# danilobellini/audiolazy

Hardware: NVIDIA H100
Metric: samples/sec through 64-ch gammatone bank (higher is better)
Workload: dtype f64

## Files before the change

### audiolazy_b200/csrc/alz_capi.cu

```cuda
#pragma GCC visibility push(default)
#include "../../include/alz_b200.h"
#pragma GCC visibility pop
#include "alz_biquad.cuh"
#include "alz_generic.cuh"
#include "alz_lane_tma.cuh"
#include "alz_plan.h"

#include <algorithm>
#include <cctype>
#include <cmath>
#include <cstring>
#include <map>
#include <thread>

#include <sys/mman.h>
#include <sys/syscall.h>
#include <unistd.h>

static std::mutex g_host_mu;
static std::map<void*, size_t> g_host_allocs;

static_assert(ALZI_OK == ALZ_OK && ALZI_ERR_CUDA == ALZ_ERR_CUDA && ALZI_ERR_UNSUPPORTED == ALZ_ERR_UNSUPPORTED, "status codes");

static thread_local std::string g_err;
std::atomic<long long> alzi_launches{0};
#define g_launches alzi_launches

int alzi_fail(int code, const char* fmt, ...) {
  char buf[512];
  va_list ap;
  va_start(ap, fmt);
  vsnprintf(buf, sizeof buf, fmt, ap);
  va_end(ap);
  g_err = buf;
  return code;
}
#define fail alzi_fail

int alzi_env_int(const char* name, int dflt) {
  const char* v = getenv(name);
  return (v && *v) ? atoi(v) : dflt;
}
#define env_int alzi_env_int

static double env_double(const char* name, double dflt) {
  const char* v = getenv(name);
  return (v && *v) ? atof(v) : dflt;
}

void alzi_keep_async_pool() {
  static std::once_flag once[64];
  int dev = 0;
  cudaGetDevice(&dev);
  std::call_once(once[dev & 63], [dev] {
    cudaMemPool_t pool;
    if (cudaDeviceGetDefaultMemPool(&pool, dev) == cudaSuccess) {
      unsigned long long keep = ~0ull;
      cudaMemPoolSetAttribute(pool, cudaMemPoolAttrReleaseThreshold, &keep);
    }
    cudaGetLastError();
  });
}
#define keep_async_pool alzi_keep_async_pool

static const int kCoefSmall = 512, kCoefLarge = 3584;

__global__ void __launch_bounds__(32)
alz_generic_kernel(const __grid_constant__ AlzTileArgs a, const __grid_constant__ AlzGenericArgs ca) {
  extern __shared__ __align__(16) float alz_smem[];
  alz_run_warp<AlzGenericCore>(a, ca, alz_smem);
}

__global__ void __launch_bounds__(32)
alz_generic_tma_kernel(const __grid_constant__ AlzTileArgs a, const __grid_constant__ AlzGenericArgs ca,
                       const __grid_constant__ CUtensorMap tmx, const __grid_constant__ CUtensorMap tmy) {
  extern __shared__ __align__(1024) unsigned char alz_smem_tma[];
  alz_run_warp_tma<AlzGenericCore>(a, ca, &tmx, &tmy, alz_smem_tma);
}

typedef CUresult (*alz_encode_tiled_fn)(CUtensorMap*, CUtensorMapDataType, cuuint32_t, void*, const cuuint64_t*,
                                        const cuuint64_t*, const cuuint32_t*, const cuuint32_t*, CUtensorMapInterleave,
                                        CUtensorMapSwizzle, CUtensorMapL2promotion, CUtensorMapFloatOOBfill);
static alz_encode_tiled_fn get_encode_tiled() {
  static alz_encode_tiled_fn fn = nullptr;
  static std::once_flag once;
  std::call_once(once, [] {
    void* p = nullptr;
    cudaDriverEntryPointQueryResult q;
    if (cudaGetDriverEntryPoint("cuTensorMapEncodeTiled", &p, cudaEnableDefault, &q) == cudaSuccess &&
        q == cudaDriverEntryPointSuccess)
      fn = (alz_encode_tiled_fn)p;
    cudaGetLastError();
  });
  return fn;
}

template <class F>
static bool driver_fn(const char* name, F* out) {
  void* p = nullptr;
  cudaDriverEntryPointQueryResult q;
  if (cudaGetDriverEntryPoint(name, &p, cudaEnableDefault, &q) != cudaSuccess || q != cudaDriverEntryPointSuccess || !p) {
    cudaGetLastError();
    return false;
  }
  *out = (F)p;
  return true;
}
static std::map<void*, CUgreenCtx> g_partitions;

bool alzi_make_tensor_maps(const AlzTileArgs& ta, CUtensorMap* tmx, CUtensorMap* tmy) {
  alz_encode_tiled_fn enc = get_encode_tiled();
  if (!enc || !ta.vec_in || !ta.vec_out || env_int("ALZ_NO_TMA", 0)) return false;
  if (ta.T >= (1ll << 31) || ta.S >= (1ll << 31)) return false;
  if ((unsigned long long)ta.xs * 4 >= (1ull << 40) || (unsigned long long)ta.ysS * 4 >= (1ull << 40)) return false;
  if (ta.ysS & 3) return false;
  const cuuint32_t estr[4] = {1, 1, 1, 1};
  if (ta.vP > 0) {
    const cuuint64_t P = (cuuint64_t)ta.vP, Sreal = (cuuint64_t)(ta.S / ta.vP);
    const cuuint64_t xdims[3] = {(cuuint64_t)ta.T, P, Sreal};
    const cuuint64_t xstr[2] = {(cuuint64_t)ta.T * 4, (cuuint64_t)ta.xs * 4};
    const cuuint32_t xbox[3] = {32, 32, 1};
    if (enc(tmx, CU_TENSOR_MAP_DATA_TYPE_FLOAT32, 3, (void*)ta.x, xdims, xstr, xbox, estr, CU_TENSOR_MAP_INTERLEAVE_NONE,
            CU_TENSOR_MAP_SWIZZLE_128B, CU_TENSOR_MAP_L2_PROMOTION_L2_128B, CU_TENSOR_MAP_FLOAT_OOB_FILL_NONE) != CUDA_SUCCESS)
      return false;
    const cuuint64_t ydims[4] = {(cuuint64_t)ta.T, P, (cuuint64_t)ta.C, Sreal};
    const cuuint64_t ystr[3] = {(cuuint64_t)ta.T * 4, (cuuint64_t)ta.ys * 4, (cuuint64_t)ta.ysS * 4};
    const cuuint32_t ybox[4] = {32, 32, 1, 1};
    return enc(tmy, CU_TENSOR_MAP_DATA_TYPE_FLOAT32, 4, (void*)ta.y, ydims, ystr, ybox, estr, CU_TENSOR_MAP_INTERLEAVE_NONE,
               CU_TENSOR_MAP_SWIZZLE_128B, CU_TENSOR_MAP_L2_PROMOTION_NONE, CU_TENSOR_MAP_FLOAT_OOB_FILL_NONE) == CUDA_SUCCESS;
  }
  {
    const cuuint64_t dims[3] = {(cuuint64_t)ta.T, (cuuint64_t)ta.S, 1};
    const cuuint64_t strides[2] = {(cuuint64_t)ta.xs * 4, (cuuint64_t)ta.xs * 4};
    const cuuint32_t box[3] = {32, 32, 1};
    if (enc(tmx, CU_TENSOR_MAP_DATA_TYPE_FLOAT32, 3, (void*)ta.x, dims, strides, box, estr, CU_TENSOR_MAP_INTERLEAVE_NONE,
            CU_TENSOR_MAP_SWIZZLE_128B, CU_TENSOR_MAP_L2_PROMOTION_L2_128B, CU_TENSOR_MAP_FLOAT_OOB_FILL_NONE) != CUDA_SUCCESS)
      return false;
  }
  {
    const cuuint64_t dims[4] = {(cuuint64_t)ta.T, (cuuint64_t)ta.C, (cuuint64_t)ta.S, 1};
    const cuuint64_t strides[3] = {(cuuint64_t)ta.ys * 4, (cuuint64_t)ta.ysS * 4, (cuuint64_t)ta.ysS * 4};
    const cuuint32_t box[4] = {32, 1, 32, 1};
    if (enc(tmy, CU_TENSOR_MAP_DATA_TYPE_FLOAT32, 4, (void*)ta.y, dims, strides, box, estr, CU_TENSOR_MAP_INTERLEAVE_NONE,
            CU_TENSOR_MAP_SWIZZLE_128B, CU_TENSOR_MAP_L2_PROMOTION_NONE, CU_TENSOR_MAP_FLOAT_OOB_FILL_NONE) != CUDA_SUCCESS)
      return false;
  }
  return true;
}

static bool make_map_2d(const float* ptr, long long T, long long n_rows, long long stride, CUtensorMap* tm) {
  alz_encode_tiled_fn enc = get_encode_tiled();
  if (!enc || ((uintptr_t)ptr & 15) || (stride & 3) || T >= (1ll << 31) || n_rows >= (1ll << 31)) return false;
  const cuuint32_t estr[2] = {1, 1};
  const cuuint64_t dims[2] = {(cuuint64_t)T, (cuuint64_t)n_rows};
  const cuuint64_t strides[1] = {(cuuint64_t)stride * 4};
  const cuuint32_t box[2] = {32, 32};
  return enc(tm, CU_TENSOR_MAP_DATA_TYPE_FLOAT32, 2, (void*)ptr, dims, strides, box, estr, CU_TENSOR_MAP_INTERLEAVE_NONE,
             CU_TENSOR_MAP_SWIZZLE_128B, CU_TENSOR_MAP_L2_PROMOTION_L2_128B, CU_TENSOR_MAP_FLOAT_OOB_FILL_NONE) == CUDA_SUCCESS;
}

static int launch_biquad(const alz_plan* p, const AlzTileArgs& ta, cudaStream_t st) {
  if (p->NB0 == 8) {
    if (p->K == 1) return alzi_launch_headfir_k1(p, ta, st);
    if (p->K == 4) return alzi_launch_headfir_k4(p, ta, st);
    return fail(ALZ_ERR_UNSUPPORTED, "no head-FIR kernel for K=%d", p->K);
  }
  switch (p->K) {
    case 1: return alzi_launch_biquad_k1(p, ta, st);
    case 2: return alzi_launch_biquad_k2(p, ta, st);
    case 3: return alzi_launch_biquad_k3(p, ta, st);
    case 4: return alzi_launch_biquad_k4(p, ta, st);
    case 6: return alzi_launch_biquad_k6(p, ta, st);
    case 8: return alzi_launch_biquad_k8(p, ta, st);
  }
  return fail(ALZ_ERR_UNSUPPORTED, "no biquad kernel for K=%d", p->K);
}

static double probe_biquad(const alz_plan* p, const double* r64, const double* r32) {
  if (p->NB0 == 8) return p->K == 1 ? alzi_probe_headfir_k1(p, r64, r32) : alzi_probe_headfir_k4(p, r64, r32);
  switch (p->K) {
    case 1: return alzi_probe_biquad_k1(p, r64, r32);
    case 2: return alzi_probe_biquad_k2(p, r64, r32);
    case 3: return alzi_probe_biquad_k3(p, r64, r32);
    case 4: return alzi_probe_biquad_k4(p, r64, r32);
    case 6: return alzi_probe_biquad_k6(p, r64, r32);
    default: return alzi_probe_biquad_k8(p, r64, r32);
  }
}

static int launch_generic(const alz_plan* p, AlzTileArgs ta, cudaStream_t st, const double* tv = nullptr,
                          long long tv_stride = 0) {
  AlzGenericArgs ga{p->d_sec, p->d_tap_delay, p->d_coef, p->K, p->C, 0, tv, tv_stride};
  const long long groups = (ta.S + 31) / 32;
  CUtensorMap tmx, tmy;
  if (alzi_make_tensor_maps(ta, &tmx, &tmy))
    alz_generic_tma_kernel<<<dim3((unsigned)p->C, (unsigned)groups), 32, ALZ_TMA_SMEM, st>>>(ta, ga, tmx, tmy);
  else
    alz_generic_kernel<<<dim3((unsigned)p->C, (unsigned)groups), 32, ALZ_WARP_SMEM, st>>>(ta, ga);
  ALZ_CUDA(cudaGetLastError());
  g_launches.fetch_add(1, std::memory_order_relaxed);
  return ALZ_OK;
}

static const int kBiquadKs[] = {1, 2, 3, 4, 6, 8};
static const double kTierMaxRadius = 0.99;
static const double kChunkMaxErr = 2.5e-8;
static const long long kChunkProbeLen = 1024;

template <class Sec>
static double chunk_error(const std::vector<Sec>& secs, long long L) {
  const size_t K = secs.size();
  struct Hist { std::vector<std::vector<double>> x, y; };
  auto zero = [&]() {
    Hist h;
    for (const Sec& s : secs) { h.x.emplace_back(s.b.size() - 1, 0.0); h.y.emplace_back(s.a.size() - 1, 0.0); }
    return h;
  };
  auto step = [&](Hist& h, double v) {
    for (size_t k = 0; k < K; ++k) {
      const Sec& s = secs[k];
      std::vector<double>& xh = h.x[k];
      std::vector<double>& yh = h.y[k];
      double acc = s.b[0] * v;
      for (size_t j = 1; j < s.b.size(); ++j) acc += s.b[j] * xh[j - 1];
      for (size_t j = 1; j < s.a.size(); ++j) acc -= s.a[j] * yh[j - 1];
      if (!xh.empty()) { std::copy_backward(xh.begin(), xh.end() - 1, xh.end()); xh[0] = v; }
      if (!yh.empty()) { std::copy_backward(yh.begin(), yh.end() - 1, yh.end()); yh[0] = acc; }
      v = acc;
    }
    return v;
  };
  std::vector<double> x(3 * L);
  unsigned seed = 2024u;
  for (auto& v : x) { seed = seed * 1664525u + 1013904223u; v = (double)(float)((double)(seed >> 8) * (2.0 / 16777216.0) - 1.0); }
  Hist seq = zero();
  for (long long n = 0; n < L; ++n) step(seq, x[n]);
  Hist chunk = seq;
  for (long long n = 0; n < L; ++n) step(chunk, 0.0);
  Hist f = zero();
  for (long long n = L; n < 2 * L; ++n) { step(seq, x[n]); step(f, x[n]); }
  for (size_t k = 0; k < K; ++k) {
    for (size_t j = 0; j < chunk.x[k].size(); ++j) chunk.x[k][j] += f.x[k][j];
    for (size_t j = 0; j < chunk.y[k].size(); ++j) chunk.y[k][j] += f.y[k][j];
  }
  double peak = 0.0, err = 0.0;
  for (long long n = 2 * L; n < 3 * L; ++n) {
    const double want = step(seq, x[n]), got = step(chunk, x[n]);
    peak = std::max(peak, std::fabs(want));
    const double d = std::fabs(got - want);
    err = std::max(err, d == d ? d : 1e300);
  }
  return peak > 0.0 ? err / peak : (err > 0.0 ? 1e300 : 0.0);
}

extern "C" {

const char* alz_last_error(void) { return g_err.c_str(); }
int32_t alz_abi_version(void) { return ALZ_ABI_VERSION; }
int64_t alz_launch_count(void) { return g_launches.load(); }

int32_t alz_device_count(void) {
  int n = 0;
  if (cudaGetDeviceCount(&n) != cudaSuccess) { cudaGetLastError(); return 0; }
  return n;
}

int32_t alz_set_device(int32_t device) {
  ALZ_CUDA(cudaSetDevice(device));
  return ALZ_OK;
}

int32_t alz_plan_create(const double* coef, const int32_t* desc, int32_t C, int32_t KM, alz_plan** out) {
  return alz_plan_create_ex(coef, desc, C, KM, 0, out);
}

int32_t alz_plan_create_ex(const double* coef, const int32_t* desc, int32_t C, int32_t KM, int32_t flags,
                           alz_plan** out) {
  if (!out) return fail(ALZ_ERR_INVALID, "out is null");
  *out = nullptr;
  if (!coef || !desc || C <= 0 || KM < 0) return fail(ALZ_ERR_INVALID, "bad plan arguments");
  const bool design_only = (flags & ALZ_PLAN_DESIGN_ONLY) != 0;
  int dev = -1;
  if (!design_only) ALZ_CUDA(cudaGetDevice(&dev));

  struct Sec { std::vector<double> b, a; };
  std::vector<std::vector<Sec>> secs(C);
  int Kmax = 0, nbmax = 1, namax = 1;
  for (int c = 0; c < C; ++c) {
    bool ended = false;
    for (int k = 0; k < KM; ++k) {
      const int32_t* d = desc + ((size_t)c * KM + k) * 3;
      const int nb = d[0], na = d[1];
      if (nb == 0) { ended = true; continue; }
      if (ended) return fail(ALZ_ERR_INVALID, "channel %d: section %d follows an absent section", c, k);
      if (nb < 0 || na < 1 || d[2] < 0) return fail(ALZ_ERR_INVALID, "channel %d section %d: bad descriptor", c, k);
      const double* b = coef + d[2];
      const double* a = b + nb;
      if (a[0] == 0.0) return fail(ALZ_ERR_ZERO_GAIN, "channel %d section %d: Invalid filter gain (a0 == 0)", c, k);
      Sec s;
      s.b.assign(b, b + nb);
      s.a.assign(a, a + na);
      const double a0 = a[0];
      if (a0 != 1.0) {
        for (auto& v : s.b) v /= a0;
        for (auto& v : s.a) v /= a0;
        s.a[0] = 1.0;
      }
      while (s.b.size() > 1 && s.b.back() == 0.0) s.b.pop_back();
      while (s.a.size() > 1 && s.a.back() == 0.0) s.a.pop_back();
      for (double v : s.b) if (!std::isfinite(v)) return fail(ALZ_ERR_INVALID, "non-finite coefficient");
      for (double v : s.a) if (!std::isfinite(v)) return fail(ALZ_ERR_INVALID, "non-finite coefficient");
      nbmax = std::max(nbmax, (int)s.b.size());
      namax = std::max(namax, (int)s.a.size());
      secs[c].push_back(std::move(s));
    }
    Kmax = std::max(Kmax, (int)secs[c].size());
  }
  if (Kmax == 0) Kmax = 1;

  alz_plan* p = new (std::nothrow) alz_plan();
  if (!p) return fail(ALZ_ERR_NOMEM, "out of host memory");
  p->C = C;
  p->device = dev;
  p->sequential = (flags & ALZ_PLAN_SEQUENTIAL) != 0;
  p->parallel_sum = (flags & ALZ_PLAN_PARALLEL) != 0;
  if (design_only || cudaDeviceGetAttribute(&p->sm_count, cudaDevAttrMultiProcessorCount, dev) != cudaSuccess || p->sm_count <= 0) {
    cudaGetLastError();
    p->sm_count = 132;
  }

  p->fr_desc.assign((size_t)C * Kmax * 3, 0);
  for (int c = 0; c < C; ++c)
    for (size_t k = 0; k < secs[c].size(); ++k) {
      int* d = &p->fr_desc[((size_t)c * Kmax + k) * 3];
      d[0] = (int)secs[c][k].b.size(); d[1] = (int)secs[c][k].a.size(); d[2] = (int)p->fr_coef.size();
      p->fr_coef.insert(p->fr_coef.end(), secs[c][k].b.begin(), secs[c][k].b.end());
      p->fr_coef.insert(p->fr_coef.end(), secs[c][k].a.begin(), secs[c][k].a.end());
    }
  p->fr_K = Kmax;

  int nb_first = 1, nb_rest = 1;
  for (int c = 0; c < C; ++c)
    for (size_t k = 0; k < secs[c].size(); ++k) {
      if (k == 0) nb_first = std::max(nb_first, (int)secs[c][k].b.size());
      else nb_rest = std::max(nb_rest, (int)secs[c][k].b.size());
    }
  const bool plain = nbmax <= 3 && namax <= 3 && Kmax <= 8;
  const bool headfir = !plain && namax <= 3 && nb_first <= 8 && nb_rest <= 3 && Kmax <= 4;
  const bool biquad = (plain || headfir) && !(flags & ALZ_PLAN_FORCE_GENERIC);
  if (biquad) {
    int K = 8;
    for (int kk : kBiquadKs) if (kk >= Kmax) { K = kk; break; }
    if (headfir) K = Kmax == 1 ? 1 : 4;
    p->kind = ALZ_KIND_BIQUAD;
    p->K = K;
    p->NB = headfir ? (nb_rest <= 1 ? 1 : 3) : nbmax;
    p->NB0 = headfir ? 8 : 0;
    p->xd = ALZ_H0(p->NB0); p->yd = 2;
    p->state_doubles = ALZ_STATE_SLOTS(K, p->NB0);
    bool monic = !p->parallel_sum;
    for (int c = 0; c < C && monic; ++c) {
      double g = 1.0;
      for (auto& s : secs[c]) {
        const double b0 = s.b[0];
        if (!(std::fabs(b0) > 1e-150 && std::fabs(b0) < 1e150)) { monic = false; break; }
        g *= b0;
        if (!(std::fabs(g) > 1e-250 && std::fabs(g) < 1e250)) { monic = false; break; }
      }
    }
    bool gain_in = monic && !env_int("ALZ_EXACT_GAIN", 0);
    for (int c = 0; c < C && gain_in; ++c) {
      double g = 1.0;
      for (auto& s : secs[c]) g *= s.b[0];
      if (!(std::fabs(g) > 1e-30 && std::fabs(g) < 1e30)) gain_in = false;
    }
    p->monic = monic ? (gain_in ? 2 : 1) : 0;
    p->fp64_ops = (monic ? K * (p->NB - 1 + 2) + (gain_in ? 0 : 1) : K * (p->NB + 2)) + (headfir ? 8 - p->NB : 0);
    if (!headfir && !env_int("ALZ_NO_ZMASK", 0)) {
      int zm = (1 << (2 * K)) - 1;
      for (int c = 0; c < C; ++c)
        for (size_t k = 0; k < secs[c].size(); ++k)
          for (int j = 1; j <= 2; ++j)
            if ((int)secs[c][k].b.size() > j && secs[c][k].b[j] != 0.0) zm &= ~(1 << (2 * (int)k + j - 1));
      p->zmask = zm;
      if (K == 4 && p->NB == 3 && (zm & ALZ_ZMASK_KLAPURI) == ALZ_ZMASK_KLAPURI) p->fp64_ops -= 6;
    }
    const int stride = ALZ_COEF_STRIDE(K, p->NB0), nval = ALZ_COEF_NVAL(K, p->NB0);
    std::vector<double> tab((size_t)C * stride, 0.0);
    p->sc.assign((size_t)C * (K + 1), 1.0);
    for (int c = 0; c < C; ++c) {
      double* rec = tab.data() + (size_t)c * stride;
      double g = 1.0, sc = 1.0;
      if (p->monic == 2) {
        double gg = 1.0;
        for (auto& s : secs[c]) gg *= s.b[0];
        sc = (double)(float)gg;
        p->sc[(size_t)c * (K + 1)] = sc;
      }
      for (int k = 0; k < K; ++k) {
        double b[8] = {1.0, 0, 0, 0, 0, 0, 0, 0}, a[3] = {1.0, 0.0, 0.0};
        if (k < (int)secs[c].size()) {
          const Sec& s = secs[c][k];
          b[0] = 0.0;
          for (size_t i = 0; i < s.b.size(); ++i) b[i] = s.b[i];
          for (size_t i = 0; i < s.a.size(); ++i) a[i] = s.a[i];
        }
        if (k == 0 && p->NB0 == 8)
          for (int j = 3; j < 8; ++j) rec[5 * K + 1 + (j - 3)] = monic ? b[j] / b[0] : b[j];
        if (monic) {
          rec[5 * k + 0] = 1.0;
          rec[5 * k + 1] = b[1] / b[0];
          rec[5 * k + 2] = b[2] / b[0];
          g *= b[0];
          sc /= b[0];
        } else {
          rec[5 * k + 0] = b[0];
          rec[5 * k + 1] = b[1];
          rec[5 * k + 2] = b[2];
        }
        rec[5 * k + 3] = -a[1];
        rec[5 * k + 4] = -a[2];
        p->sc[(size_t)c * (K + 1) + k + 1] = sc;
      }
      rec[5 * K] = monic ? g : 1.0;
    }
    p->tier.assign(C, 0);
    p->tier_err.assign(C, -1.0);
    p->tier_tol = env_double("ALZ_TIER_TOL", 2.5e-6);
    p->probe_len = std::max(64, env_int("ALZ_TIER_PROBE", 8192));
    const bool tiering = !(flags & ALZ_PLAN_EXACT) && !p->parallel_sum && !env_int("ALZ_NO_FP32_TIER", 0) && p->tier_tol > 0.0;
    std::vector<double> tab32((size_t)C * stride, 0.0);
    for (int c = 0; c < C; ++c) {
      const double* rec = tab.data() + (size_t)c * stride;
      float* r32 = reinterpret_cast<float*>(tab32.data() + (size_t)c * stride);
      bool representable = true;
      for (int i = 0; i < nval; ++i) {
        r32[i] = (float)rec[i];
        if (rec[i] != 0.0 && !(std::fabs(rec[i]) > 1e-30 && std::fabs(rec[i]) < 1e30)) representable = false;
      }
      double radius = 0.0;
      for (auto& s : secs[c]) {
        const double a1 = s.a.size() > 1 ? s.a[1] : 0.0, a2 = s.a.size() > 2 ? s.a[2] : 0.0, disc = a1 * a1 - 4.0 * a2;
        radius = std::max(radius, disc < 0.0 ? std::sqrt(a2) : 0.5 * (std::fabs(a1) + std::sqrt(disc)));
      }
      if (tiering && representable) {
        p->tier_err[c] = probe_biquad(p, rec, tab32.data() + (size_t)c * stride);
        if (p->tier_err[c] <= p->tier_tol && radius <= kTierMaxRadius) { p->tier[c] = 1; ++p->n_fp32; }
      }
    }
    if (!p->sequential)
      for (int c = 0; c < C; ++c) p->chunk_err = std::max(p->chunk_err, chunk_error(secs[c], kChunkProbeLen));
    {
      std::vector<int> lst[2];
      const int order = env_int("ALZ_TIER_ORDER", 1);
      for (int c = 0; c < C; ++c) lst[order == 1 ? p->tier[c] : (order == 2 ? 1 - p->tier[c] : 0)].push_back(c);
      size_t i0 = 0, i1 = 0;
      p->pos_channel.clear();
      while (i0 < lst[0].size() || i1 < lst[1].size()) {
        const bool take0 = i1 >= lst[1].size() || (i0 < lst[0].size() && i0 * lst[1].size() <= i1 * lst[0].size());
        p->pos_channel.push_back(take0 ? lst[0][i0++] : lst[1][i1++]);
      }
    }
    p->h_tab.assign((size_t)C * stride, 0.0);
    for (int pos = 0; pos < C; ++pos) {
      const int c = p->pos_channel[pos];
      const std::vector<double>& src = p->tier[c] ? tab32 : tab;
      double* rec = p->h_tab.data() + (size_t)pos * stride;
      memcpy(rec, src.data() + (size_t)c * stride, (size_t)nval * sizeof(double));
      rec[ALZ_COEF_META(K, p->NB0)] = (double)(c + 65536 * p->tier[c]);
    }
    p->fp64_ops_exact = p->fp64_ops;
    p->coef_small = C * stride <= kCoefSmall;
    const int ncoef = p->coef_small ? kCoefSmall : kCoefLarge;
    const int per_launch = ncoef / stride;
    if (per_launch < 1) { alz_plan_destroy(p); return fail(ALZ_ERR_UNSUPPORTED, "coefficient record too large"); }
    for (int p0 = 0; p0 < C; p0 += per_launch) {
      const int npos = std::min(per_launch, C - p0);
      char* blk = (char*)calloc(1, 2 * sizeof(int) + (size_t)ncoef * sizeof(double));
      if (!blk) { alz_plan_destroy(p); return fail(ALZ_ERR_NOMEM, "out of host memory"); }
      reinterpret_cast<int*>(blk)[0] = stride;
      reinterpret_cast<int*>(blk)[1] = npos;
      memcpy(blk + 2 * sizeof(int), p->h_tab.data() + (size_t)p0 * stride, (size_t)npos * stride * sizeof(double));
      p->chunks.push_back({blk, npos});
    }
    p->tile_group = env_int("ALZ_TILE_GROUP", 2);
    if (p->tile_group != 1 && p->tile_group != 2 && p->tile_group != 4) p->tile_group = 2;
  } else if (Kmax == 1 && !(flags & ALZ_PLAN_FORCE_GENERIC) && C * 32 <= kCoefLarge && !env_int("ALZ_NO_WINDOW", 0)) {
    p->kind = ALZ_KIND_GENERIC;
    p->window = true;
    p->K = 1;
    p->NB = nbmax;
    p->monic = 0;
    int near_x = 0, near_y = 0, maxd_x = 0, maxd_y = 0;
    std::vector<int> far_x, far_y;
    for (int c = 0; c < C; ++c) {
      if (secs[c].empty()) continue;
      const Sec& s = secs[c][0];
      for (size_t d = 1; d < s.b.size(); ++d)
        if (s.b[d] != 0.0) {
          maxd_x = std::max(maxd_x, (int)d);
          if (d < 16) near_x = std::max(near_x, (int)d);
          else if (std::find(far_x.begin(), far_x.end(), (int)d) == far_x.end()) far_x.push_back((int)d);
        }
      for (size_t d = 1; d < s.a.size(); ++d)
        if (s.a[d] != 0.0) {
          maxd_y = std::max(maxd_y, (int)d);
          if (d < 16) near_y = std::max(near_y, (int)d);
          else if (std::find(far_y.begin(), far_y.end(), (int)d) == far_y.end()) far_y.push_back((int)d);
        }
    }
    std::sort(far_x.begin(), far_x.end());
    std::sort(far_y.begin(), far_y.end());
    auto slots_of = [](int nearest) { return nearest == 0 ? 0 : (nearest <= 3 ? 4 : 16); };
    auto pow2 = [](int n) { int q = 1; while (q < n) q <<= 1; return q; };
    p->win_mx = slots_of(near_x);
    p->win_my = slots_of(near_y);
    p->win_nfx = (int)far_x.size();
    p->win_nfy = (int)far_y.size();
    int slot = 1;
    p->win_xwin = slot; slot += p->win_mx ? p->win_mx - 1 : 0;
    p->win_ywin = slot; slot += p->win_my ? p->win_my - 1 : 0;
    if (!far_x.empty()) { p->win_xbase = slot; p->win_xmask = pow2(far_x.back() + 16) - 1; slot += p->win_xmask + 1; }
    if (!far_y.empty()) { p->win_ybase = slot; p->win_ymask = pow2(far_y.back() + 16) - 1; slot += p->win_ymask + 1; }
    p->xd = maxd_x; p->yd = maxd_y;
    p->state_doubles = slot;
    p->fp64_ops = 1 + (p->win_mx ? p->win_mx - 1 : 0) + (p->win_my ? p->win_my - 1 : 0) + p->win_nfx + p->win_nfy;
    p->win_far_delay = far_x;
    p->win_far_delay.insert(p->win_far_delay.end(), far_y.begin(), far_y.end());
    p->h_tab.assign((size_t)C * 32, 0.0);
    std::vector<double> fcoef(std::max<size_t>(1, p->win_far_delay.size()) * C, 0.0);
    for (int c = 0; c < C; ++c) {
      double* rec = p->h_tab.data() + (size_t)c * 32;
      if (secs[c].empty()) { rec[0] = 1.0; continue; }
      const Sec& s = secs[c][0];
      for (size_t d = 0; d < s.b.size() && d < 16; ++d) rec[d] = s.b[d];
      for (size_t d = 1; d < s.a.size() && d < 16; ++d) rec[16 + d - 1] = -s.a[d];
      for (size_t f = 0; f < far_x.size(); ++f) fcoef[f * C + c] = (size_t)far_x[f] < s.b.size() ? s.b[far_x[f]] : 0.0;
      for (size_t f = 0; f < far_y.size(); ++f) fcoef[(far_x.size() + f) * C + c] = (size_t)far_y[f] < s.a.size() ? -s.a[far_y[f]] : 0.0;
    }
    p->coef_small = C * 32 <= 64;
    p->win_block = calloc(1, alzi_window_block_bytes(p->coef_small));
    if (!p->win_block) { alz_plan_destroy(p); return fail(ALZ_ERR_NOMEM, "out of host memory"); }
    if (!design_only) {
      const size_t nf = std::max<size_t>(1, p->win_far_delay.size());
      std::vector<int> fd(nf, 16);
      std::copy(p->win_far_delay.begin(), p->win_far_delay.end(), fd.begin());
      cudaError_t e = cudaMalloc(&p->d_far_delay, nf * sizeof(int));
      if (e == cudaSuccess) e = cudaMemcpy(p->d_far_delay, fd.data(), nf * sizeof(int), cudaMemcpyHostToDevice);
      if (e == cudaSuccess) e = cudaMalloc(&p->d_far_coef, fcoef.size() * sizeof(double));
      if (e == cudaSuccess) e = cudaMemcpy(p->d_far_coef, fcoef.data(), fcoef.size() * sizeof(double), cudaMemcpyHostToDevice);
      if (e != cudaSuccess) { alz_plan_destroy(p); return fail(ALZ_ERR_CUDA, "plan upload failed: %s", cudaGetErrorString(e)); }
    }
    alzi_window_block_fill(p->win_block, p->coef_small, p->win_nfx, p->win_nfy, p->win_xbase, p->win_xmask, p->win_ybase,
                           p->win_ymask, p->win_xwin, p->win_ywin, C, p->d_far_delay, p->d_far_coef, p->h_tab.data());
  } else {
    const int K = Kmax;
    p->kind = ALZ_KIND_GENERIC;
    p->K = K;
    p->NB = nbmax;
    p->monic = 0;
    std::vector<int> tap_delay;
    std::vector<std::vector<double>> tap_coef;
    p->h_sec.resize(K);
    p->h_xlen.assign(K, 0);
    p->h_ylen.assign(K, 0);
    int slot = 1;
    int ops = 0, xdmax = 0, ydmax = 0;
    for (int k = 0; k < K; ++k) {
      size_t nb = 1, na = 1;
      for (int c = 0; c < C; ++c)
        if (k < (int)secs[c].size()) { nb = std::max(nb, secs[c][k].b.size()); na = std::max(na, secs[c][k].a.size()); }
      AlzGenSection gs{};
      gs.num_begin = (int)tap_delay.size();
      for (size_t d = 0; d < nb; ++d) {
        std::vector<double> col(C, 0.0);
        bool any = false;
        for (int c = 0; c < C; ++c) {
          double v;
          if (k < (int)secs[c].size()) v = d < secs[c][k].b.size() ? secs[c][k].b[d] : 0.0;
          else v = d == 0 ? 1.0 : 0.0;
          col[c] = v;
          any = any || v != 0.0;
        }
        if (any || d == 0) { tap_delay.push_back((int)d); tap_coef.push_back(std::move(col)); p->h_tap_is_den.push_back(0); }
      }
      gs.nnum = (int)tap_delay.size() - gs.num_begin;
      gs.den_begin = (int)tap_delay.size();
      for (size_t d = 1; d < na; ++d) {
        std::vector<double> col(C, 0.0);
        bool any = false;
        for (int c = 0; c < C; ++c) {
          double v = (k < (int)secs[c].size() && d < secs[c][k].a.size()) ? -secs[c][k].a[d] : 0.0;
          col[c] = v;
          any = any || v != 0.0;
        }
        if (any) { tap_delay.push_back((int)d); tap_coef.push_back(std::move(col)); p->h_tap_is_den.push_back(1); }
      }
      gs.nden = (int)tap_delay.size() - gs.den_begin;
      const int xlen = (int)nb - 1, ylen = (int)na - 1;
      auto pow2 = [](int n) { int q = 1; while (q < n) q <<= 1; return q; };
      if (xlen > 0) { gs.xbase = slot; gs.xmask = pow2(xlen) - 1; slot += gs.xmask + 1; } else { gs.xbase = 0; gs.xmask = -1; }
      if (ylen > 0) { gs.ybase = slot; gs.ymask = pow2(ylen) - 1; slot += gs.ymask + 1; } else { gs.ybase = 0; gs.ymask = -1; }
      p->h_sec[k] = gs;
      p->h_xlen[k] = xlen;
      p->h_ylen[k] = ylen;
      xdmax = std::max(xdmax, xlen);
      ydmax = std::max(ydmax, ylen);
      ops += gs.nnum + gs.nden;
    }
    p->xd = xdmax; p->yd = ydmax;
    p->state_doubles = slot;
    p->fp64_ops = ops;
    const size_t ntaps = tap_delay.size();
    p->h_tap_delay = tap_delay;
    std::vector<double> tab(ntaps * C);
    for (size_t t = 0; t < ntaps; ++t) memcpy(&tab[t * C], tap_coef[t].data(), C * sizeof(double));
    cudaError_t e = design_only ? cudaSuccess : cudaMalloc(&p->d_coef, tab.size() * sizeof(double));
    if (design_only) { *out = p; return ALZ_OK; }
    if (e == cudaSuccess) e = cudaMemcpy(p->d_coef, tab.data(), tab.size() * sizeof(double), cudaMemcpyHostToDevice);
    if (e == cudaSuccess) e = cudaMalloc(&p->d_sec, K * sizeof(AlzGenSection));
    if (e == cudaSuccess) e = cudaMemcpy(p->d_sec, p->h_sec.data(), K * sizeof(AlzGenSection), cudaMemcpyHostToDevice);
    if (e == cudaSuccess) e = cudaMalloc(&p->d_tap_delay, ntaps * sizeof(int));
    if (e == cudaSuccess) e = cudaMemcpy(p->d_tap_delay, tap_delay.data(), ntaps * sizeof(int), cudaMemcpyHostToDevice);
    if (e != cudaSuccess) { alz_plan_destroy(p); return fail(ALZ_ERR_CUDA, "plan upload failed: %s", cudaGetErrorString(e)); }
  }
  *out = p;
  return ALZ_OK;
}

void alz_plan_destroy(alz_plan* p) {
  if (!p) return;
  if (p->device < 0) {
    for (auto& ch : p->chunks) free(ch.block);
    free(p->win_block);
    delete p;
    return;
  }
  int cur = 0;
  cudaGetDevice(&cur);
  cudaSetDevice(p->device);
  cudaDeviceSynchronize();
  if (p->pipe.ready) {
    for (int i = 0; i < AlzHostPipe::NBUF; ++i) {
      if (p->pipe.stream[i]) { cudaStreamSynchronize(p->pipe.stream[i]); cudaStreamDestroy(p->pipe.stream[i]); }
      if (p->pipe.done[i]) cudaEventDestroy(p->pipe.done[i]);
      cudaFree(p->pipe.dx[i]);
      cudaFree(p->pipe.dy[i]);
      cudaFree(p->pipe.dst[i]);
      cudaFree(p->pipe.des[i]);
    }
  }
  for (auto& ch : p->chunks) free(ch.block);
  for (auto* e : p->m_cache) { cudaFree(e->M); cudaEventDestroy(e->ready); delete e; }
  free(p->win_block);
  cudaFree(p->d_far_delay);
  cudaFree(p->d_far_coef);
  cudaFree(p->d_coef);
  cudaFree(p->d_sec);
  cudaFree(p->d_tap_delay);
  cudaFree(p->d_fr_coef);
  cudaFree(p->d_fr_desc);
  cudaSetDevice(cur);
  cudaGetLastError();
  delete p;
}

int32_t alz_plan_info_get(const alz_plan* p, alz_plan_info* out) {
  if (!p || !out) return fail(ALZ_ERR_INVALID, "null argument");
  memset(out, 0, sizeof *out);
  out->abi_version = ALZ_ABI_VERSION;
  out->kind = p->kind;
  out->n_channels = p->C;
  out->n_sections = p->K;
  out->num_taps = p->NB0 ? p->NB0 : p->NB;
  out->monic = p->monic;
  out->state_doubles = p->state_doubles;
  out->fp64_ops = p->fp64_ops;
  out->device = p->device;
  out->n_fp32_channels = p->n_fp32;
  out->tier_tol_e9 = (int32_t)std::min(2.0e9, p->tier_tol * 1e9 + 0.5);
  out->time_parallel = p->kind == ALZ_KIND_BIQUAD && !p->sequential && p->chunk_err <= kChunkMaxErr;
  return ALZ_OK;
}

int32_t alz_plan_tiers(const alz_plan* p, int32_t* tier, double* probe_err, int32_t cap) {
  if (!p) return fail(ALZ_ERR_INVALID, "plan is null");
  for (int c = 0; c < p->C && c < cap; ++c) {
    const bool have = c < (int)p->tier.size();
    if (tier) tier[c] = have ? p->tier[c] : 0;
    if (probe_err) probe_err[c] = have ? p->tier_err[c] : -1.0;
  }
  return p->C;
}

int64_t alz_plan_state_doubles(const alz_plan* p, int64_t S) {
  if (!p || S < 0) return fail(ALZ_ERR_INVALID, "bad argument");
  return (int64_t)p->state_doubles * S * p->C;
}

int32_t alz_plan_history(const alz_plan* p, int32_t* xd, int32_t* yd) {
  if (!p || !xd || !yd) return fail(ALZ_ERR_INVALID, "null argument");
  *xd = p->xd;
  *yd = p->yd;
  return ALZ_OK;
}

static __global__ void alz_state_fill_kernel(double* state, const double* proto, long long R, int C, int slots) {
  const long long i = (long long)blockIdx.x * blockDim.x + threadIdx.x;
  if (i >= R * slots) return;
  const long long slot = i / R, r = i - slot * R, S = R / C;
  state[i] = proto[slot * C + (int)(r / S)];
}

int32_t alz_state_init(const alz_plan* p, double* state, int64_t S, const double* xinit, const double* yinit,
                       void* cuda_stream) {
  if (!p || S < 0) return fail(ALZ_ERR_INVALID, "bad argument");
  if (p->device < 0) return fail(ALZ_ERR_CUDA, "design-only plan: no device");
  if (S == 0) return ALZ_OK;
  if (!state) return fail(ALZ_ERR_INVALID, "state is null");
  cudaStream_t st = (cudaStream_t)cuda_stream;
  const long long R = (long long)S * p->C;
  const size_t bytes = (size_t)p->state_doubles * R * sizeof(double);
  if (!xinit && !yinit) {
    ALZ_CUDA(cudaMemsetAsync(state, 0, bytes, st));
    return ALZ_OK;
  }
  const int C = p->C, K = p->K, slots = p->state_doubles;
  std::vector<double> proto((size_t)slots * C, 0.0);
  if (p->kind == ALZ_KIND_BIQUAD) {
    for (int c = 0; c < C; ++c)
      for (int k = 0; k < K; ++k) {
        const double sc_in = p->sc[(size_t)c * (K + 1) + k], sc_out = p->sc[(size_t)c * (K + 1) + k + 1];
        const int base = ALZ_STATE_BASE(k, p->NB0);
        const int nx = k == 0 ? ALZ_H0(p->NB0) : 2;
        for (int j = 0; j < nx; ++j) {
          const double xv = xinit ? xinit[((size_t)c * K + k) * p->xd + j] : 0.0;
          proto[(size_t)(base + j) * C + c] = (p->monic == 2 && k == 0) ? (double)((float)xv * (float)sc_in) : xv * sc_in;
        }
        for (int j = 0; j < 2; ++j) {
          const double yv = yinit ? yinit[((size_t)c * K + k) * 2 + j] : 0.0;
          proto[(size_t)(base + nx + j) * C + c] = yv * sc_out;
        }
      }
  } else if (p->window) {
    for (int c = 0; c < C; ++c) {
      for (int j = 0; j < p->xd; ++j) {
        const double xv = xinit ? xinit[(size_t)c * p->xd + j] : 0.0;
        if (j + 1 < p->win_mx) proto[(size_t)(p->win_xwin + j) * C + c] = xv;
        if (p->win_xmask >= 0) proto[(size_t)(p->win_xbase + ((-(j + 1)) & p->win_xmask)) * C + c] = xv;
      }
      for (int j = 0; j < p->yd; ++j) {
        const double yv = yinit ? yinit[(size_t)c * p->yd + j] : 0.0;
        if (j + 1 < p->win_my) proto[(size_t)(p->win_ywin + j) * C + c] = yv;
        if (p->win_ymask >= 0) proto[(size_t)(p->win_ybase + ((-(j + 1)) & p->win_ymask)) * C + c] = yv;
      }
    }
  } else {
    for (int c = 0; c < C; ++c)
      for (int k = 0; k < K; ++k) {
        const AlzGenSection& gs = p->h_sec[k];
        for (int j = 0; j < p->h_xlen[k]; ++j) {
          const double xv = xinit ? xinit[((size_t)c * K + k) * p->xd + j] : 0.0;
          proto[(size_t)(gs.xbase + ((-(j + 1)) & gs.xmask)) * C + c] = xv;
        }
        for (int j = 0; j < p->h_ylen[k]; ++j) {
          const double yv = yinit ? yinit[((size_t)c * K + k) * p->yd + j] : 0.0;
          proto[(size_t)(gs.ybase + ((-(j + 1)) & gs.ymask)) * C + c] = yv;
        }
      }
  }
  double* d_proto = nullptr;
  ALZ_CUDA(cudaMallocAsync((void**)&d_proto, proto.size() * sizeof(double), st));
  ALZ_CUDA(cudaMemcpyAsync(d_proto, proto.data(), proto.size() * sizeof(double), cudaMemcpyHostToDevice, st));
  const long long n = R * slots;
  alz_state_fill_kernel<<<(unsigned)((n + 255) / 256), 256, 0, st>>>(state, d_proto, R, C, slots);
  ALZ_CUDA(cudaGetLastError());
  g_launches.fetch_add(1, std::memory_order_relaxed);
  ALZ_CUDA(cudaFreeAsync(d_proto, st));
  ALZ_CUDA(cudaStreamSynchronize(st));
  return ALZ_OK;
}

static int apply_launch(const alz_plan* p, AlzTileArgs ta, double* state, long long sstride, cudaStream_t st,
                        const double* tv, long long tv_stride) {
  ta.state = state;
  ta.sstride = sstride;
  if (p->kind == ALZ_KIND_BIQUAD) return launch_biquad(p, ta, st);
  if (p->window) return alzi_launch_window(p, ta, st);
  return launch_generic(p, ta, st, tv, tv_stride);
// ... 843 lines not shown
```

### audiolazy_b200/csrc/alz_launch.cuh

```cuda
#pragma once
#include <algorithm>
#include <cmath>
#include <cstring>

#include "alz_biquad.cuh"
#include "alz_lane_tma.cuh"
#include "alz_plan.h"

static const int kCoefSmall = 512, kCoefLarge = 3584;
static const int kWarpsPerSm = 22;
static const int kWarpsPerSmTma = 24;

template <int K, int NB, int MONIC, int NCOEF, int NB0, int ZMASK>
__global__ void __launch_bounds__(32, kWarpsPerSm)
alz_biquad_kernel(const __grid_constant__ AlzTileArgs a, const __grid_constant__ AlzBiquadArgs<NCOEF> ca) {
  extern __shared__ __align__(16) float alz_smem[];
  if (ca.tier(blockIdx.x) == 0) alz_run_warp<AlzBiquadCore<K, NB, MONIC, NB0, ZMASK, double>>(a, ca, alz_smem);
  else alz_run_warp<AlzBiquadCore<K, NB, MONIC, NB0, ZMASK, float>>(a, ca, alz_smem);
}

template <int K, int NB, int MONIC, int NCOEF, int NB0, int ZMASK>
__global__ void __launch_bounds__(32, kWarpsPerSmTma)
alz_biquad_tma_kernel(const __grid_constant__ AlzTileArgs a, const __grid_constant__ AlzBiquadArgs<NCOEF> ca,
                      const __grid_constant__ CUtensorMap tmx, const __grid_constant__ CUtensorMap tmy) {
  extern __shared__ __align__(1024) unsigned char alz_smem_tma[];
  if (ca.tier(blockIdx.x) == 0)
    alz_run_warp_tma<AlzBiquadCore<K, NB, MONIC, NB0, ZMASK, double>>(a, ca, &tmx, &tmy, alz_smem_tma);
  else
    alz_run_warp_tma<AlzBiquadCore<K, NB, MONIC, NB0, ZMASK, float>>(a, ca, &tmx, &tmy, alz_smem_tma);
}

template <int K, int NB, int MONIC, int NCOEF, int NB0, int ZMASK>
__global__ void __launch_bounds__(32, kWarpsPerSmTma)
alz_biquad_envelope_kernel(const __grid_constant__ AlzTileArgs a, const __grid_constant__ AlzBiquadArgs<NCOEF> ca,
                           const __grid_constant__ CUtensorMap tmx, const __grid_constant__ CUtensorMap tmy) {
  extern __shared__ __align__(1024) unsigned char alz_smem_tma[];
  if (ca.tier(blockIdx.x) == 0)
    alz_run_warp_tma<AlzBiquadCore<K, NB, MONIC, NB0, ZMASK, double>, AlzEnvelopePost>(a, ca, &tmx, &tmy, alz_smem_tma);
  else
    alz_run_warp_tma<AlzBiquadCore<K, NB, MONIC, NB0, ZMASK, float>, AlzEnvelopePost>(a, ca, &tmx, &tmy, alz_smem_tma);
}

template <int K, int NB, int NB0, int ZMASK>
static int launch_envelope_t(const alz_plan* p, AlzTileArgs ta, cudaStream_t st) {
  if (p->coef_small || p->chunks.size() != 1)
    return alzi_fail(ALZI_ERR_UNSUPPORTED, "envelope consumer: gammatone-bank plans only");
  CUtensorMap tmx, tmy;
  if (!alzi_make_tensor_maps(ta, &tmx, &tmy)) return alzi_fail(ALZI_ERR_UNSUPPORTED, "envelope consumer needs 16-byte aligned x rows");
  const long long groups = (ta.S + 31) / 32;
  ta.paired = (long long)p->chunks[0].npos * groups >= (long long)p->sm_count * kWarpsPerSmTma ? 2 : 1;
  ta.groups = (int)groups;
  void* args[4] = {(void*)&ta, p->chunks[0].block, (void*)&tmx, (void*)&tmy};
  const void* kern = p->monic == 2 ? (const void*)alz_biquad_envelope_kernel<K, NB, 2, kCoefLarge, NB0, ZMASK>
                   : p->monic == 1 ? (const void*)alz_biquad_envelope_kernel<K, NB, 1, kCoefLarge, NB0, ZMASK>
                                   : (const void*)alz_biquad_envelope_kernel<K, NB, 0, kCoefLarge, NB0, ZMASK>;
  ALZ_CUDA(cudaLaunchKernel(kern, dim3((unsigned)p->chunks[0].npos, (unsigned)groups), dim3(32), args, ALZ_TMA_SMEM_FOR(ta.paired), st));
  ALZ_CUDA(cudaGetLastError());
  alzi_launches.fetch_add(1, std::memory_order_relaxed);
  return ALZI_OK;
}

template <int K, int NB, int MONIC, int NCOEF, int NB0, int ZMASK>
static int launch_biquad_chunk(const alz_plan* p, AlzTileArgs ta, const void* block, int npos, cudaStream_t st) {
  const long long groups = (ta.S + 31) / 32;
  CUtensorMap tmx, tmy;
  if (alzi_make_tensor_maps(ta, &tmx, &tmy)) {
    const long long warps = (long long)npos * groups;
    int ng = warps >= (long long)p->sm_count * kWarpsPerSmTma ? p->tile_group : 1;
    ng = alzi_env_int("ALZ_TMA_PAIRED", ng);
    if (ng != 2 && ng != 4) ng = 1;
    ta.paired = ng;
    ta.exp |= alzi_env_int("ALZ_EXP", 0);
    const size_t smem = ALZ_TMA_SMEM_FOR(ng);
    const long long per_sm = std::min<long long>(kWarpsPerSmTma, (228 * 1024) / (long long)(smem + 1024));
    const long long slots = (long long)p->sm_count * per_sm;
    long long nseg = 1;
    if (ta.vP == 0 && warps > slots && warps < 8 * slots && ta.T >= 2048 && !alzi_env_int("ALZ_NO_SEGMENT", 0)) {
      const long long waves = std::max(1, alzi_env_int("ALZ_SEG_WAVES", 16)), min_len = std::max(32, alzi_env_int("ALZ_SEG_MIN", 1024));
      nseg = std::min((waves * slots + warps - 1) / warps, ta.T / min_len);
      const long long quantum = 32ll * ng;
      const long long len = ((ta.T + nseg - 1) / nseg + quantum - 1) / quantum * quantum;
      nseg = (ta.T + len - 1) / len;
      if (nseg > 1 && groups * nseg <= 65535) {
        const size_t words = (size_t)npos + (size_t)npos * groups;
        unsigned* sync = nullptr;
        alzi_keep_async_pool();
        ALZ_CUDA(cudaMallocAsync(&sync, words * 4, st));
        if (cudaMemsetAsync(sync, 0, words * 4, st) != cudaSuccess) {
          cudaFreeAsync(sync, st);
          ALZ_CUDA(cudaGetLastError());
        }
        ta.nseg = (int)nseg; ta.seg_len = len; ta.sync = sync;
      } else {
        nseg = 1;
      }
    }
    ta.groups = (int)groups;
    auto kern = alz_biquad_tma_kernel<K, NB, MONIC, NCOEF, NB0, ZMASK>;
    if (smem > 48 * 1024) return alzi_fail(ALZI_ERR_UNSUPPORTED, "tile group too large");
    void* args[4] = {(void*)&ta, const_cast<void*>(block), (void*)&tmx, (void*)&tmy};
    const cudaError_t e = cudaLaunchKernel((const void*)kern, dim3((unsigned)npos, (unsigned)(groups * nseg)), dim3(32), args, smem, st);
    if (ta.sync) cudaFreeAsync(ta.sync, st);
    ALZ_CUDA(e);
  } else {
    if (ta.exp & 2) ta.y = nullptr;
    auto kern = alz_biquad_kernel<K, NB, MONIC, NCOEF, NB0, ZMASK>;
    void* args[2] = {(void*)&ta, const_cast<void*>(block)};
    ALZ_CUDA(cudaLaunchKernel((const void*)kern, dim3((unsigned)npos, (unsigned)groups), dim3(32), args, ALZ_WARP_SMEM, st));
  }
  ALZ_CUDA(cudaGetLastError());
  alzi_launches.fetch_add(1, std::memory_order_relaxed);
  return ALZI_OK;
}

template <int K, int NB, int MONIC, int NB0, int ZMASK>
static int launch_biquad_t(const alz_plan* p, const AlzTileArgs& ta, cudaStream_t st) {
  for (const auto& ch : p->chunks) {
    const int rc = p->coef_small ? launch_biquad_chunk<K, NB, MONIC, kCoefSmall, NB0, ZMASK>(p, ta, ch.block, ch.npos, st)
                                 : launch_biquad_chunk<K, NB, MONIC, kCoefLarge, NB0, ZMASK>(p, ta, ch.block, ch.npos, st);
    if (rc != ALZI_OK) return rc;
  }
  return ALZI_OK;
}

template <int K, int NB, int NB0, int ZMASK = 0>
static int launch_biquad_nb(const alz_plan* p, const AlzTileArgs& ta, cudaStream_t st) {
  if (p->monic == 2) return launch_biquad_t<K, NB, 2, NB0, ZMASK>(p, ta, st);
  if (p->monic == 1) return launch_biquad_t<K, NB, 1, NB0, ZMASK>(p, ta, st);
  return launch_biquad_t<K, NB, 0, NB0, ZMASK>(p, ta, st);
}

template <int K>
static int launch_biquad_k(const alz_plan* p, const AlzTileArgs& ta, cudaStream_t st) {
  switch (p->NB) {
    case 1: return launch_biquad_nb<K, 1, 0>(p, ta, st);
    case 2: return launch_biquad_nb<K, 2, 0>(p, ta, st);
    default:
      if constexpr (K == 4) {
        if ((p->zmask & ALZ_ZMASK_KLAPURI) == ALZ_ZMASK_KLAPURI) return launch_biquad_nb<4, 3, 0, ALZ_ZMASK_KLAPURI>(p, ta, st);
      }
      return launch_biquad_nb<K, 3, 0>(p, ta, st);
  }
}

template <int K>
static int launch_headfir_k(const alz_plan* p, const AlzTileArgs& ta, cudaStream_t st) {
  if constexpr (K == 1) return launch_biquad_nb<1, 1, 8>(p, ta, st);
  else {
    if (p->NB <= 1) return launch_biquad_nb<K, 1, 8>(p, ta, st);
    return launch_biquad_nb<K, 3, 8>(p, ta, st);
  }
}

static inline float alzi_probe_noise(unsigned& s) {
  s = s * 1664525u + 1013904223u;
  return (float)((double)(s >> 8) * (2.0 / 16777216.0) - 1.0);
}

template <int K, int NB, int MONIC, int NB0, int ZMASK>
static double probe_biquad_t(const double* rec64, const double* rec32, int n) {
  double worst = 0.0;
  for (int sig = 0; sig < 5; ++sig) {
    AlzBiquadCore<K, NB, MONIC, NB0, ZMASK, double> c64;
    AlzBiquadCore<K, NB, MONIC, NB0, ZMASK, float> c32;
    c64.load_coef(rec64); c64.zero_state();
    c32.load_coef(rec32); c32.zero_state();
    unsigned seed = 12345u;
    double peak = 0.0, err = 0.0;
    for (int i = 0; i < n; ++i) {
      const float nyq = (i & 1) ? -1.0f : 1.0f;
      const float x = sig == 0 ? alzi_probe_noise(seed) : sig == 1 ? 1.0f : sig == 2 ? (i == 0 ? 1.0f : 0.0f)
                      : sig == 3 ? 0.5f * alzi_probe_noise(seed) + 0.5f * nyq : nyq;
      float y64, y32;
      if (i < 2) { y64 = c64.step_explicit(c64.widen(x)); y32 = c32.step_explicit(c32.widen(x)); }
      else { y64 = c64.step_alias(c64.widen(x)); y32 = c32.step_alias(c32.widen(x)); }
      peak = std::max(peak, std::fabs((double)y64));
      const double d = std::fabs((double)y32 - (double)y64);
      err = std::max(err, d == d ? d : 1e300);
    }
    if (peak > 0.0) worst = std::max(worst, err / peak);
    else if (err > 0.0) worst = 1e300;
  }
  return worst;
}

template <int K, int NB, int NB0, int ZMASK = 0>
static double probe_biquad_nb(const alz_plan* p, const double* r64, const double* r32, int n) {
  if (p->monic == 2) return probe_biquad_t<K, NB, 2, NB0, ZMASK>(r64, r32, n);
  if (p->monic == 1) return probe_biquad_t<K, NB, 1, NB0, ZMASK>(r64, r32, n);
  return probe_biquad_t<K, NB, 0, NB0, ZMASK>(r64, r32, n);
}

template <int K>
static double probe_biquad_k(const alz_plan* p, const double* r64, const double* r32) {
  const int n = p->probe_len;
  switch (p->NB) {
    case 1: return probe_biquad_nb<K, 1, 0>(p, r64, r32, n);
    case 2: return probe_biquad_nb<K, 2, 0>(p, r64, r32, n);
    default:
      if constexpr (K == 4) {
        if ((p->zmask & ALZ_ZMASK_KLAPURI) == ALZ_ZMASK_KLAPURI) return probe_biquad_nb<4, 3, 0, ALZ_ZMASK_KLAPURI>(p, r64, r32, n);
      }
      return probe_biquad_nb<K, 3, 0>(p, r64, r32, n);
  }
}

template <int K>
static double probe_headfir_k(const alz_plan* p, const double* r64, const double* r32) {
  if constexpr (K == 1) return probe_biquad_nb<1, 1, 8>(p, r64, r32, p->probe_len);
  else {
    if (p->NB <= 1) return probe_biquad_nb<K, 1, 8>(p, r64, r32, p->probe_len);
    return probe_biquad_nb<K, 3, 8>(p, r64, r32, p->probe_len);
  }
}
```

### audiolazy_b200/csrc/alz_plan.h

```cpp
#pragma once
#include <cuda.h>
#include <cuda_runtime.h>
#include <atomic>
#include <cstdarg>
#include <cstdio>
#include <cstdlib>
#include <cstring>
#include <mutex>
#include <string>
#include <vector>

#include "alz_generic.cuh"
#include "alz_lane.cuh"

#define ALZI_OK 0
#define ALZI_ERR_CUDA (-4)
#define ALZI_ERR_UNSUPPORTED (-6)

int alzi_fail(int code, const char* fmt, ...);
int alzi_env_int(const char* name, int dflt);
void alzi_keep_async_pool();
extern std::atomic<long long> alzi_launches;

#define ALZ_CUDA(expr)                                                                        \
  do {                                                                                        \
    cudaError_t e__ = (expr);                                                                 \
    if (e__ != cudaSuccess)                                                                   \
      return alzi_fail(ALZI_ERR_CUDA, "%s failed: %s (%s:%d)", #expr, cudaGetErrorString(e__), __FILE__, __LINE__); \
  } while (0)

struct AlzHostPipe {
  static const int NBUF = 4;
  cudaStream_t stream[NBUF] = {};
  cudaEvent_t done[NBUF] = {};
  float* dx[NBUF] = {};
  float* dy[NBUF] = {};
  double* dst[NBUF] = {};
  double* des[NBUF] = {};
  size_t dx_bytes = 0, dy_bytes = 0, dst_bytes = 0, des_bytes = 0;
  bool ready = false;
};

struct alz_plan {
  int kind = 0, C = 0, K = 0, NB = 0, NB0 = 0, monic = 0, device = 0, sm_count = 132;
  int zmask = 0;
  int xd = 0, yd = 0;
  int state_doubles = 0;
  int fp64_ops = 0;
  int fp64_ops_exact = 0;
  int n_fp32 = 0;
  double tier_tol = 0.0;
  int probe_len = 8192;
  int tile_group = 2;
  bool parallel_sum = false;
  bool sequential = false;
  double chunk_err = 0.0;
  bool coef_small = false;
  struct Chunk { void* block; int npos; };
  std::vector<Chunk> chunks;
  bool window = false;
  int win_mx = 0, win_my = 0;
  int win_xwin = 0, win_ywin = 0;
  int win_xbase = 0, win_xmask = -1, win_ybase = 0, win_ymask = -1;
  std::vector<int> win_far_delay;
  int win_nfx = 0, win_nfy = 0;
  void* win_block = nullptr;
  int* d_far_delay = nullptr;
  double* d_far_coef = nullptr;
  double* d_coef = nullptr;
  AlzGenSection* d_sec = nullptr;
  int* d_tap_delay = nullptr;
  std::vector<double> h_tab;
  std::vector<int> pos_channel;
  std::vector<int> tier;
  std::vector<double> tier_err;
  std::vector<double> sc;
  std::vector<AlzGenSection> h_sec;
  std::vector<int> h_xlen, h_ylen;
  std::vector<int> h_tap_delay, h_tap_is_den;
  std::vector<double> fr_coef;
  std::vector<int> fr_desc;
  double* d_fr_coef = nullptr;
  int fr_K = 0;
  int* d_fr_desc = nullptr;
  struct MEntry { long long L; double* M; cudaEvent_t ready; int users; bool evicted; };
  std::mutex m_mu;
  std::vector<MEntry*> m_cache;
  std::mutex host_mu;
  AlzHostPipe pipe;
};

int alzi_launch_biquad_k1(const alz_plan*, const AlzTileArgs&, cudaStream_t);
int alzi_launch_biquad_k2(const alz_plan*, const AlzTileArgs&, cudaStream_t);
int alzi_launch_biquad_k3(const alz_plan*, const AlzTileArgs&, cudaStream_t);
int alzi_launch_biquad_k4(const alz_plan*, const AlzTileArgs&, cudaStream_t);
int alzi_launch_biquad_k6(const alz_plan*, const AlzTileArgs&, cudaStream_t);
int alzi_launch_biquad_k8(const alz_plan*, const AlzTileArgs&, cudaStream_t);
int alzi_launch_headfir_k1(const alz_plan*, const AlzTileArgs&, cudaStream_t);
int alzi_launch_headfir_k4(const alz_plan*, const AlzTileArgs&, cudaStream_t);

int alzi_launch_envelope_k4(const alz_plan*, const AlzTileArgs&, cudaStream_t);
int alzi_launch_envelope_headfir_k4(const alz_plan*, const AlzTileArgs&, cudaStream_t);
int alzi_launch_window(const alz_plan*, const AlzTileArgs&, cudaStream_t);
int alzi_launch_parallel(const alz_plan*, const AlzTileArgs&, const CUtensorMap& tmx, const CUtensorMap& tmo, cudaStream_t);
size_t alzi_window_block_bytes(bool small);
void alzi_window_block_fill(void* blk, bool small, int n_far_x, int n_far_y, int xbase, int xmask, int ybase, int ymask, int xwin,
                            int ywin, int C, const int* far_delay, const double* far_coef, const double* coef);

double alzi_probe_biquad_k1(const alz_plan*, const double* rec64, const double* rec32);
double alzi_probe_biquad_k2(const alz_plan*, const double* rec64, const double* rec32);
double alzi_probe_biquad_k3(const alz_plan*, const double* rec64, const double* rec32);
double alzi_probe_biquad_k4(const alz_plan*, const double* rec64, const double* rec32);
double alzi_probe_biquad_k6(const alz_plan*, const double* rec64, const double* rec32);
double alzi_probe_biquad_k8(const alz_plan*, const double* rec64, const double* rec32);
double alzi_probe_headfir_k1(const alz_plan*, const double* rec64, const double* rec32);
double alzi_probe_headfir_k4(const alz_plan*, const double* rec64, const double* rec32);

bool alzi_make_tensor_maps(const AlzTileArgs& ta, CUtensorMap* tmx, CUtensorMap* tmy);
```

Before: 9.466 billion.

## Pick tile group and segment count from measured occupancy and tail idle

Chooses tile group 4 by default when the per-sample FP64 op count is small, and replaces the hard-coded CTAs-per-SM estimate with a cached cudaOccupancy query after setting the max-shared carveout. Segment count is now chosen by searching for the split that minimises idle slots in the last wave, not from a fixed wave target. The aim is better SM fill and less tail imbalance for the gammatone bank. The risks are extra sync-buffer allocation and launch-time work when segmenting, and possibly worse performance from the larger tile group.

```diff
diff --git a/audiolazy_b200/csrc/alz_capi.cu b/audiolazy_b200/csrc/alz_capi.cu
--- a/audiolazy_b200/csrc/alz_capi.cu
+++ b/audiolazy_b200/csrc/alz_capi.cu
@@ -206,6 +206,7 @@
 static const double kTierMaxRadius = 0.99;
 static const double kChunkMaxErr = 2.5e-8;
 static const long long kChunkProbeLen = 1024;
+static const int kTileGroup4MaxFp64 = 16;
 
 template <class Sec>
 static double chunk_error(const std::vector<Sec>& secs, long long L) {
@@ -483,8 +484,9 @@
       memcpy(blk + 2 * sizeof(int), p->h_tab.data() + (size_t)p0 * stride, (size_t)npos * stride * sizeof(double));
       p->chunks.push_back({blk, npos});
     }
-    p->tile_group = env_int("ALZ_TILE_GROUP", 2);
-    if (p->tile_group != 1 && p->tile_group != 2 && p->tile_group != 4) p->tile_group = 2;
+    const int group = env_int("ALZ_TILE_GROUP", 0);
+    p->tile_group_forced = group == 1 || group == 2 || group == 4;
+    p->tile_group = p->tile_group_forced ? group : (p->fp64_ops <= kTileGroup4MaxFp64 ? 4 : 2);
   } else if (Kmax == 1 && !(flags & ALZ_PLAN_FORCE_GENERIC) && C * 32 <= kCoefLarge && !env_int("ALZ_NO_WINDOW", 0)) {
     p->kind = ALZ_KIND_GENERIC;
     p->window = true;
diff --git a/audiolazy_b200/csrc/alz_launch.cuh b/audiolazy_b200/csrc/alz_launch.cuh
--- a/audiolazy_b200/csrc/alz_launch.cuh
+++ b/audiolazy_b200/csrc/alz_launch.cuh
@@ -10,6 +10,7 @@
 static const int kCoefSmall = 512, kCoefLarge = 3584;
 static const int kWarpsPerSm = 22;
 static const int kWarpsPerSmTma = 24;
+static const double kSegTailIdle = 0.02;
 
 template <int K, int NB, int MONIC, int NCOEF, int NB0, int ZMASK>
 __global__ void __launch_bounds__(32, kWarpsPerSm)
@@ -60,46 +61,76 @@
   return ALZI_OK;
 }
 
+static int tma_ctas_per_sm(const alz_plan* p, const void* kern, int ng, long long* out) {
+  std::atomic<int>& cached = p->tma_ctas_per_sm[ng >= 4 ? 1 : 0];
+  int n = cached.load(std::memory_order_relaxed);
+  if (n == 0) {
+    ALZ_CUDA(cudaFuncSetAttribute(kern, cudaFuncAttributePreferredSharedMemoryCarveout, cudaSharedmemCarveoutMaxShared));
+    ALZ_CUDA(cudaOccupancyMaxActiveBlocksPerMultiprocessor(&n, kern, 32, ALZ_TMA_SMEM_FOR(ng)));
+    if (n < 1) return alzi_fail(ALZI_ERR_UNSUPPORTED, "bank kernel: no CTA of %d tiles fits on an SM", ng < 2 ? 2 : ng);
+    cached.store(n, std::memory_order_relaxed);
+  }
+  *out = n;
+  return ALZI_OK;
+}
+
 template <int K, int NB, int MONIC, int NCOEF, int NB0, int ZMASK>
 static int launch_biquad_chunk(const alz_plan* p, AlzTileArgs ta, const void* block, int npos, cudaStream_t st) {
   const long long groups = (ta.S + 31) / 32;
   CUtensorMap tmx, tmy;
   if (alzi_make_tensor_maps(ta, &tmx, &tmy)) {
+    const void* kern = (const void*)alz_biquad_tma_kernel<K, NB, MONIC, NCOEF, NB0, ZMASK>;
     const long long warps = (long long)npos * groups;
-    int ng = warps >= (long long)p->sm_count * kWarpsPerSmTma ? p->tile_group : 1;
+    const long long min_len = std::max(32, alzi_env_int("ALZ_SEG_MIN", 1024));
+    const bool can_segment = ta.vP == 0 && ta.T >= 2 * min_len && !alzi_env_int("ALZ_NO_SEGMENT", 0);
+    long long per_one = 0, per_group = 0;
+    int rc = tma_ctas_per_sm(p, kern, 1, &per_one);
+    if (rc == ALZI_OK) rc = tma_ctas_per_sm(p, kern, p->tile_group, &per_group);
+    if (rc != ALZI_OK) return rc;
+    const bool fills = warps >= p->sm_count * per_group && (can_segment || warps >= p->sm_count * per_one);
+    int ng = p->tile_group_forced || fills ? p->tile_group : 1;
     ng = alzi_env_int("ALZ_TMA_PAIRED", ng);
     if (ng != 2 && ng != 4) ng = 1;
     ta.paired = ng;
     ta.exp |= alzi_env_int("ALZ_EXP", 0);
     const size_t smem = ALZ_TMA_SMEM_FOR(ng);
-    const long long per_sm = std::min<long long>(kWarpsPerSmTma, (228 * 1024) / (long long)(smem + 1024));
+    long long per_sm = 0;
+    if ((rc = tma_ctas_per_sm(p, kern, ng, &per_sm)) != ALZI_OK) return rc;
     const long long slots = (long long)p->sm_count * per_sm;
-    long long nseg = 1;
-    if (ta.vP == 0 && warps > slots && warps < 8 * slots && ta.T >= 2048 && !alzi_env_int("ALZ_NO_SEGMENT", 0)) {
-      const long long waves = std::max(1, alzi_env_int("ALZ_SEG_WAVES", 16)), min_len = std::max(32, alzi_env_int("ALZ_SEG_MIN", 1024));
-      nseg = std::min((waves * slots + warps - 1) / warps, ta.T / min_len);
+    auto idle = [&](long long n) {
+      const long long cap = (n * warps + slots - 1) / slots * slots;
+      return (double)(cap - n * warps) / (double)cap;
+    };
+    long long nseg = 1, len = ta.T;
+    if (can_segment && warps > slots && idle(1) > kSegTailIdle) {
       const long long quantum = 32ll * ng;
-      const long long len = ((ta.T + nseg - 1) / nseg + quantum - 1) / quantum * quantum;
-      nseg = (ta.T + len - 1) / len;
-      if (nseg > 1 && groups * nseg <= 65535) {
-        const size_t words = (size_t)npos + (size_t)npos * groups;
-        unsigned* sync = nullptr;
-        alzi_keep_async_pool();
-        ALZ_CUDA(cudaMallocAsync(&sync, words * 4, st));
-        if (cudaMemsetAsync(sync, 0, words * 4, st) != cudaSuccess) {
-          cudaFreeAsync(sync, st);
-          ALZ_CUDA(cudaGetLastError());
-        }
-        ta.nseg = (int)nseg; ta.seg_len = len; ta.sync = sync;
-      } else {
-        nseg = 1;
-      }
+      double best = idle(1);
+      for (long long n = 2; n <= ta.T / min_len && groups * n <= 65535; ++n) {
+        const long long ln = ((ta.T + n - 1) / n + quantum - 1) / quantum * quantum;
+        if ((ta.T + ln - 1) / ln != n) continue;
+        const double f = idle(n);
+        if (f < best) { best = f; nseg = n; len = ln; }
+        if (f <= kSegTailIdle) break;
+      }
+    }
+    if (alzi_env_int("ALZ_LOG_LAUNCH", 0))
+      fprintf(stderr, "alz bank launch: %lld warps, tile group %d, %lld CTAs per SM (%lld slots), %lld segment(s) of %lld samples\n",
+              warps, ng, per_sm, slots, nseg, len);
+    if (nseg > 1) {
+      const size_t words = (size_t)npos + (size_t)npos * groups;
+      unsigned* sync = nullptr;
+      alzi_keep_async_pool();
+      ALZ_CUDA(cudaMallocAsync(&sync, words * 4, st));
+      if (cudaMemsetAsync(sync, 0, words * 4, st) != cudaSuccess) {
+        cudaFreeAsync(sync, st);
+        ALZ_CUDA(cudaGetLastError());
+      }
+      ta.nseg = (int)nseg; ta.seg_len = len; ta.sync = sync;
     }
     ta.groups = (int)groups;
-    auto kern = alz_biquad_tma_kernel<K, NB, MONIC, NCOEF, NB0, ZMASK>;
     if (smem > 48 * 1024) return alzi_fail(ALZI_ERR_UNSUPPORTED, "tile group too large");
     void* args[4] = {(void*)&ta, const_cast<void*>(block), (void*)&tmx, (void*)&tmy};
-    const cudaError_t e = cudaLaunchKernel((const void*)kern, dim3((unsigned)npos, (unsigned)(groups * nseg)), dim3(32), args, smem, st);
+    const cudaError_t e = cudaLaunchKernel(kern, dim3((unsigned)npos, (unsigned)(groups * nseg)), dim3(32), args, smem, st);
     if (ta.sync) cudaFreeAsync(ta.sync, st);
     ALZ_CUDA(e);
   } else {
diff --git a/audiolazy_b200/csrc/alz_plan.h b/audiolazy_b200/csrc/alz_plan.h
--- a/audiolazy_b200/csrc/alz_plan.h
+++ b/audiolazy_b200/csrc/alz_plan.h
@@ -51,7 +51,9 @@
   int n_fp32 = 0;
   double tier_tol = 0.0;
   int probe_len = 8192;
-  int tile_group = 2;
+  int tile_group = 4;
+  bool tile_group_forced = false;
+  mutable std::atomic<int> tma_ctas_per_sm[2] = {};
   bool parallel_sum = false;
   bool sequential = false;
   double chunk_err = 0.0;
```

Result: faster. 9.838 billion, median of 6 (+3.9%).
